# iscc/iscc-search

Measured on AMD Instinct MI355X. Metric: queries/sec (+ roofline of the dominant kernel), 64-bit Hamming k=10 over 100M codes, exact top-k, higher is better.
Workload: dtype fp4 (e2m1 0/1 x +-1 products, f32 accumulation: exact integers)

## Files before the change

### iscc_search_amd/csrc/batch.hip.h

```cpp

void launch_scan(int W, bool mask, int tq, int mode, dim3 grid, hipStream_t st, const isk::ScanParams& p) {
    auto with_tq = [&](auto&& f) { if (tq == 8) f(isk::int_c<8>{}); else f(isk::int_c<16>{}); };
    if (W == 1 && !mask) {
        isk::with_mode(mode, [&](auto m) { with_tq([&](auto t) {
            if constexpr (decltype(m)::value != isk::MODE_SELF) hipLaunchKernelGGL((isk::scan_adapt_kernel<decltype(t)::value, decltype(m)::value>), grid, dim3(isk::BLOCK), 0, st, p);
        }); });
        return;
    }
    isk::with_words(W, [&](auto w) {
        auto masked = [&](auto mk) { with_tq([&](auto t) { isk::with_mode(mode, [&](auto m) {
            constexpr int WORDS = decltype(w)::value, MODE = decltype(m)::value;
            constexpr bool MASK = decltype(mk)::value;
            if constexpr (MODE != isk::MODE_SELF && (WORDS > 1 || MASK)) hipLaunchKernelGGL((isk::scan_kernel<WORDS, MASK, decltype(t)::value, MODE>), grid, dim3(isk::BLOCK), 0, st, p);
        }); }); };
        if (mask) masked(std::true_type{}); else masked(std::false_type{});
    });
}
int tile_rows_for(int W) { return W == 1 ? isk::tile_rows<1>() : W == 2 ? isk::tile_rows<2>() : W == 3 ? isk::tile_rows<3>() : isk::tile_rows<4>(); }

constexpr uint64_t CACHE_RESIDENT_BYTES = 128ull << 20;
uint32_t scan_grid_x(H* h, int W, uint64_t rows, uint32_t groups = 1, bool sample = false) {
    const uint64_t tiles = rows / (uint64_t)tile_rows_for(W);
    uint64_t maxb = (uint64_t)h->cus * BLOCKS_PER_CU;
    if (sample || rows * 8 * (uint64_t)W <= CACHE_RESIDENT_BYTES)
// ... 138 lines not shown
    bool single_pass(const Job& j) const { return allow_self && h->opt.self_tighten && use_mfma(j, j.seg->n); }
    enum class Path { tiny, radius, single, levels };
    Path path(const Job& j) const {
        if (tiny(j)) return Path::tiny;
        if (job_radius(j) >= 0) return Path::radius;
        return single_pass(j) ? Path::single : Path::levels;
    }
    bool pack3(const Job& j) const { return j.pack && h->opt.mfma_pack3 && isk::mfma_pack3_fits(isk::mfma_groups_per_chunk((int)j.W, nq_pad, j.pack)); }
    bool pack3_pass(const Job& j) const { return use_mfma(j, j.seg->n) && pack3(j); }
    int scan(const Job& j, const isk::ScanParams& sp, int mode, bool sample) {
        const uint64_t rows = sp.n_rows - sp.row_begin;
        if (use_mfma(j, rows) || mode == isk::MODE_SELF) {
            const uint32_t g = isk::mfma_groups_per_chunk((int)j.W, nq_pad, j.pack);
            const uint32_t chunks = (nq_pad + g * 32 - 1) / (g * 32);
            const bool pack3 = this->pack3(j);
            const uint64_t rps = isk::mfma_rows_per_wave_step((int)j.W, j.pack, pack3);
            const uint64_t steps = (rows + rps - 1) / rps;
            const uint64_t wpb = isk::mfma_waves_per_block();
            const uint64_t bx = std::max<uint64_t>(1, std::min<uint64_t>((steps + wpb - 1) / wpb, std::max<uint32_t>(1, (uint32_t)h->cus * isk::mfma_blocks_per_cu((int)j.W, g, j.pack) / chunks)));
            const int e = isk::launch_mfma_scan((int)j.W, mode, j.pack, (uint32_t)bx, g, h->stream, sp, pack3);
            if (e) return fail(-EIO, "mfma scan: chunk of %u query groups does not fit the LDS budget (%s)", g, hipGetErrorString((hipError_t)e));
            h->stats.mfma_launches += 1;
            if (j.pack) h->stats.mfma_pack_launches += 1;
            h->stats.mfma_pair_words += rows * (uint64_t)nq * j.W;
            return 0;
        }
        if (mode != isk::MODE_COLLECT && mode != isk::MODE_STRETCH && mode != isk::MODE_BOTH) return fail(-EINVAL, "scan mode %d has no XOR + popcount kernel", mode);
        if (sp.n_rows / (uint64_t)tile_rows_for((int)j.W) >= (1ull << 31)) return fail(-E2BIG, "segment of %llu rows exceeds the scan kernel's 2^31 tiles", (unsigned long long)sp.n_rows);
        launch_scan((int)j.W, j.mask, tq, mode, dim3(scan_grid_x(h, j.W, rows, groups, sample), groups), h->stream, sp);
        return 0;
    }

    void plan(const uint64_t* hq) {
        jobs.clear();
        tq = (int)h->opt.queries_per_pass;
        if (tq == 8 && nq > 8 && nq <= 16) tq = 16;
        nq_pad = (nq + tq - 1) / tq * tq;
        groups = nq_pad / tq;
        for (uint32_t b = 1; b <= ISCCSEARCH_MAX_BYTES; ++b) {
            Segment& s = t.seg[b];
            if (!s.n) continue;
            Job j;
            j.seg = &s;
            j.pbytes = t.metric == ISCCSEARCH_METRIC_NPHD ? std::min(b, qbytes) : b;
            j.W = (j.pbytes + 7) / 8;
            j.mask = (j.pbytes & 7) != 0;
            j.mask_last = mask_for(j.pbytes);
            j.pack = h->opt.mfma_pack && j.W == 1;
            if (j.pack && j.pbytes == 8)
                for (uint32_t q = 0; q < nq && j.pack; ++q) j.pack = hq[(size_t)q * t.max_words] != 0;
            jobs.push_back(j);
        }
    }
    int reserve() {
        cap = std::max<uint32_t>((uint32_t)h->opt.candidate_cap, 16 * k);
        if (h->opt.self_tighten && h->opt.mfma && radius < 0 && radius_ratio < 0) cap = std::max<uint32_t>(cap, 64 * k);
        multi = jobs.size() > 1;
        P = next_pow2(std::max<uint32_t>(std::max<uint32_t>(k, 1024), std::min<uint32_t>(4 * k, 4096)));
        sel_lds = (((size_t)P * 4 + 15) & ~(size_t)15) + (size_t)P * 8 * t.key_words + (d_out_rows ? (size_t)P * 4 : 0);
        int rc;
        if ((rc = h->d_queries.ensure((size_t)nq_pad * 4))) return rc;
        if ((rc = h->d_bias.ensure(nq_pad))) return rc;
        if ((rc = h->d_thr.ensure(nq_pad))) return rc;
        if ((rc = h->d_cnt.ensure((size_t)nq_pad * isk::CNT_STRIDE))) return rc;
        if ((rc = h->d_ghist.ensure((size_t)nq_pad * isk::HB))) return rc;
        if (!d_flags) {
            if ((rc = h->d_overflow.ensure(flag_words()))) return rc;
            d_flags = h->d_overflow.p;
        }
        if ((rc = h->d_cand.ensure((size_t)nq_pad * cap))) return rc;
        if (multi) {
            if ((rc = h->d_lists.ensure(jobs.size() * (size_t)nq * k))) return rc;
            if ((rc = h->d_listcnt.ensure(jobs.size() * (size_t)nq))) return rc;
        }
        return 0;
    }
    const uint64_t* staged() const { return h->p_queries.p + pq_off; }
    bool all_tiny() const {
        for (const Job& j : jobs) if (!tiny(j)) return false;
        return true;
    }
    bool inline_queries() const { return !all_tiny() && radius >= 0 && nq_pad <= isk::INLINE_QUERIES && jobs.size() == 1; }
    bool tiny_inline() const { return all_tiny() && nq_pad <= isk::INLINE_QUERIES; }
    int stage(const uint64_t* hq) {
        int rc;
        if ((rc = wait_staged(h))) return rc;
        if ((rc = h->p_queries.ensure(pq_off + (size_t)nq_pad * 4))) return rc;
        uint64_t* const pq = h->p_queries.p + pq_off;
        memset(pq, 0, (size_t)nq_pad * 4 * 8);
        for (uint32_t q = 0; q < nq; ++q)
            for (int w = 0; w < t.max_words; ++w) pq[(size_t)q * 4 + w] = hq[(size_t)q * t.max_words + w];
        if (!inline_queries() && !tiny_inline()) HIPOK(hipMemcpyAsync(h->d_queries.p, pq, (size_t)nq_pad * 4 * 8, hipMemcpyHostToDevice, h->stream));
        if (mark_overflow) { HIPOK(hipEventRecord(h->ev_staged, h->stream)); h->ev_staged_pending = true; }
        return 0;
    }
    int begin(const uint64_t* hq) {
        plan(hq);
        used_self = false;
        if (jobs.empty()) {
            HIPOK(hipMemsetAsync(d_out_cnt, 0, nq * sizeof(uint32_t), h->stream));
            return 0;
        }
        int rc;
        if ((rc = reserve())) return rc;
        if ((rc = stage(hq))) return rc;
        for (size_t ji = 0; ji < jobs.size(); ++ji) {
            Run run{jobs[ji], make_ctx(ji), job_radius(jobs[ji])};
            switch (path(run.j)) {
                case Path::tiny: rc = run_tiny(run); break;
                case Path::radius: rc = run_radius(run); break;
                case Path::single: used_self = true; rc = run_single(run); break;
                case Path::levels: rc = run_levels(run); break;
            }
            if (rc) return rc;
        }
        return 0;
    }

    void count_scan(const Job& j, uint64_t rows, uint32_t passes) {
        h->stats.scan_launches += 1;
        h->stats.scan_passes += passes;
        h->stats.scan_bytes += rows * 8 * j.W * passes;
        h->stats.scan_pair_words += rows * (uint64_t)nq * j.W;
    }
    int run_tiny(Run& run) {
        const Job& j = run.j;
        const Segment& s = *j.seg;
        isk::TinyParams tp{};
        set_cols(tp.col, s, j.W);
        tp.queries = h->d_queries.p; tp.cand = h->d_cand.p; tp.mask_last = j.mask_last; tp.n_rows = (uint32_t)s.n; tp.W = j.W;
        tp.radius = run.radius; tp.use_inline = tiny_inline() ? 1u : 0u;
        isk::InlineQueries iq;
        if (tp.use_inline) memcpy(iq.w, staged(), (size_t)nq_pad * 4 * 8);
        else memset(iq.w, 0, sizeof iq.w);
        hipEvent_t e1 = nullptr;
        int rc;
        if ((rc = profile_begin(h, e1))) return rc;
        const bool wide = (s.n > 2048 && nq <= (uint32_t)h->cus / 2) || run.c.sl.P >= 2 * (uint64_t)h->opt.select_wide_from || (run.c.sl.P >= (uint64_t)h->opt.select_wide_from && nq <= (uint32_t)h->cus / 2);
        if (wide) launch_tiny_nt<1024>(tp, run.c.sl, iq);
        else launch_tiny_nt<isk::BLOCK>(tp, run.c.sl, iq);
        HIPOK(hipGetLastError());
        if ((rc = profile_end(h, e1))) return rc;
        count_scan(j, s.n, nq);
        return 0;
    }

    int collect(Run& run, uint64_t from, bool self = false) {
        const Job& j = run.j;
        const Segment& s = *j.seg;
        isk::ScanParams& sp = run.c.sp;
        const uint64_t tile_rows = (uint64_t)tile_rows_for((int)j.W);
        uint64_t stretch = s.n;
        const bool shared = use_mfma(j, s.n - from) ? nq_pad > isk::mfma_groups_per_chunk((int)j.W, nq_pad, j.pack) * 32 : groups > 1;
        const uint64_t stretch_bytes = ((uint64_t)h->opt.stretch_mb << 20) * (use_mfma(j, s.n - from) ? (uint64_t)h->opt.mfma_stretch_factor : 1);
        if (shared && stretch_bytes) stretch = std::max<uint64_t>(tile_rows, stretch_bytes / (8 * j.W) / tile_rows * tile_rows);
        for (uint64_t a = from; a < s.n;) {
            const uint64_t b = s.n - a <= stretch + stretch / 4 ? s.n : a + stretch;
            sp.row_begin = a;
            sp.n_rows = b;
            const uint64_t rows = b - a;
            hipEvent_t e1 = nullptr;
            int rcl = 0;
            if ((rcl = profile_begin(h, e1))) return rcl;
            const bool hist_too = run.radius < 0;
            const bool repick = hist_too && b < s.n && !self;
            if (self) {
                if ((rcl = scan(j, sp, isk::MODE_SELF, false))) return rcl;
            } else if (hist_too) {
                if (!run.hist_live) { HIPOK(hipMemsetAsync(h->d_ghist.p, 0, (size_t)nq_pad * isk::HB * sizeof(uint32_t), h->stream)); run.hist_live = true; }
                if ((rcl = scan(j, sp, isk::MODE_STRETCH, false))) return rcl;
            } else {
                if ((rcl = scan(j, sp, isk::MODE_COLLECT, false))) return rcl;
            }
            if ((rcl = profile_end(h, e1))) return rcl;
            if (repick) {
                isk::PickParams pp{h->d_ghist.p, h->d_bias.p, nq, (uint32_t)std::min<uint64_t>(k, b), h->d_cnt.p, h->d_cand.p, cap};
                hipLaunchKernelGGL(isk::pick_kernel, dim3(nq), dim3(isk::BLOCK), 0, h->stream, pp);
            }
            count_scan(j, rows, groups);
            if (use_mfma(j, rows) || self) h->stats.scan_mfma_launches += 1;
            a = b;
        }
        return 0;
    }

    int run_radius(Run& run) {
        if (inline_queries()) {
            isk::InlineQueries iq;
            memcpy(iq.w, staged(), (size_t)nq_pad * 4 * 8);
            hipLaunchKernelGGL(isk::radius_init_inline_kernel, dim3(1), dim3(isk::BLOCK), 0, h->stream,
                               h->d_bias.p, h->d_cnt.p, nq, nq_pad, 0x7FFFFFFFu - (uint32_t)run.radius, h->d_queries.p, iq);
        } else
        hipLaunchKernelGGL(isk::radius_init_kernel, dim3((nq_pad + isk::BLOCK - 1) / isk::BLOCK), dim3(isk::BLOCK), 0, h->stream,
                           h->d_bias.p, h->d_cnt.p, nq, nq_pad, 0x7FFFFFFFu - (uint32_t)run.radius);
        int rc;
        if ((rc = collect(run, 0))) return rc;
        launch_select(run.c.sl, nq);
        HIPOK(hipGetLastError());
        return 0;
    }

    uint64_t sample_rows(const Job& j, bool self) const {
        const uint64_t n = j.seg->n;
        return std::min<uint64_t>(n, self ? std::max<uint64_t>(std::max<uint64_t>((uint64_t)h->opt.self_boot_rows, k), std::min<uint64_t>((uint64_t)h->opt.self_boot_per_k * k, n / 8))
                                          : std::max<uint64_t>(BOOT_ROWS, std::min<uint64_t>(65536, 64ull * k)));
    }
    void boot(Run& run, bool self) {
        const Job& j = run.j;
        isk::BootParams bp{};
        set_cols(bp.col, *j.seg, j.W);
        bp.queries = h->d_queries.p; bp.bias = h->d_bias.p; bp.cnt = h->d_cnt.p; bp.s0 = sample_rows(j, self); bp.nq = nq; bp.k = k; bp.W = j.W; bp.mask_last = j.mask_last;
        bp.thr = self ? h->d_thr.p : nullptr;
        bp.thr_packed = j.pack ? 1u : 0u;
        bp.counts = h->d_ghist.p;
        bp.hint = isk::BOOT_NO_HINT;
        run.hist_live = true;
        const int job_hint = self_hint >= 0 ? self_hint : (radius_ratio >= 0 && ratio_starts_self ? ratio_bits(j) : -1);
        if (self && job_hint >= 0) {
            bp.hint = (uint32_t)job_hint;
            used_hint = true;
            hipLaunchKernelGGL(isk::boot_kernel, dim3(nq_pad), dim3(64), 0, h->stream, bp);
        } else if (nq_pad > 64) {
            isk::with_words((int)j.W, [&](auto w) { hipLaunchKernelGGL(isk::boot_multi_kernel<decltype(w)::value>, dim3(nq_pad / isk::BOOT_QB), dim3(1024), 0, h->stream, bp); });
        } else {
            hipLaunchKernelGGL(isk::boot_kernel, dim3(nq_pad), dim3(1024), 0, h->stream, bp);
        }
    }

    int run_single(Run& run) {
        boot(run, true);
        int rc;
        if ((rc = collect(run, 0, true))) return rc;
        launch_select(run.c.sl, nq);
        HIPOK(hipGetLastError());
        return 0;
    }

    uint64_t level_growth(const Job& j) const {
        uint64_t growth = (groups <= 2 && k <= 64) ? 64 : LEVEL_GROWTH;
        if (use_mfma(j, j.seg->n) && k <= 64) growth = MFMA_LEVEL_GROWTH;
        if (k >= 256) growth = std::min<uint64_t>(growth, 2);
        while (growth > 2 && (uint64_t)k * growth * 5 / 2 > (uint64_t)cap * 9 / 10) growth /= 2;
        return growth;
    }
    int run_levels(Run& run) {
        const Job& j = run.j;
        const Segment& s = *j.seg;
        isk::ScanParams& sp = run.c.sp;
        const uint64_t tile_rows = (uint64_t)tile_rows_for((int)j.W);
        int rc;
        boot(run, false);
        const uint64_t growth = level_growth(j);
        uint64_t done = 0;
        uint64_t reach = sample_rows(j, false);
        for (;;) {
            uint64_t end = reach >= s.n / growth ? s.n : reach * growth;
            if (end < s.n) end = end / tile_rows * tile_rows;
            if (end <= done || end + tile_rows > s.n) end = s.n;
            const bool last = end == s.n;
            if (last) break;
            if (!run.hist_live) {
                HIPOK(hipMemsetAsync(h->d_ghist.p, 0, (size_t)nq_pad * isk::HB * sizeof(uint32_t), h->stream));
                run.hist_live = true;
            }
            sp.row_begin = done;
            sp.n_rows = end;
            {
                hipEvent_t e1 = nullptr;
                if ((rc = profile_begin(h, e1, true))) return rc;
                if ((rc = scan(j, sp, isk::MODE_BOTH, true))) return rc;
                if ((rc = profile_end(h, e1))) return rc;
                h->stats.level_launches += 1;
                h->stats.level_pair_words += (end - done) * (uint64_t)nq * j.W;
                if (use_mfma(j, end - done)) h->stats.level_mfma_launches += 1;
            }
            isk::PickParams pp{h->d_ghist.p, h->d_bias.p, nq, (uint32_t)std::min<uint64_t>(k, end), h->d_cnt.p, h->d_cand.p, cap};
            hipLaunchKernelGGL(isk::pick_kernel, dim3(nq), dim3(isk::BLOCK), 0, h->stream, pp);
            h->stats.sample_bytes += (end - done) * 8 * j.W * groups;
// ... 157 lines not shown
```

### iscc_search_amd/csrc/isccsearch.hip

```cpp
#include <hip/hip_runtime.h>

#include <algorithm>
#include <cerrno>
#include <cstdarg>
#include <cstdio>
#include <cmath>
#include <condition_variable>
#include <cstring>
#include <memory>
#include <mutex>
#include <string>
#include <unordered_map>
#include <thread>
#include <atomic>
#include <functional>
#include <vector>

#include "../../include/isccsearch.h"
#include "kernels.hip.h"
#include "join.hip.h"
#include "mfma_scan.h"
#include "docfreq.h"
#include "simprint_score.h"
#include "asset_score.h"
#include "overlap.h"
#include "segments.h"
#include "keymap.h"

namespace {

thread_local std::string g_last_error;

int fail(int code, const char* fmt, ...) {
    char buf[512];
    va_list ap;
    va_start(ap, fmt);
    vsnprintf(buf, sizeof buf, fmt, ap);
    va_end(ap);
    g_last_error = buf;
    return code;
}

#define HIPOK(expr)                                                                              \
    do {                                                                                         \
        hipError_t e_ = (expr);                                                                  \
        if (e_ != hipSuccess) {                                                                  \
            (void)hipGetLastError();                                                             \
            return fail(e_ == hipErrorOutOfMemory ? -ENOMEM : -EIO, "%s failed: %s (%s:%d)", #expr, \
                        hipGetErrorString(e_), __FILE__, __LINE__);                              \
        }                                                                                        \
    } while (0)

using iskhost::Key;
using iskhost::KeyHash;
using iskhost::KeyMap;
using iskhost::Loc;

struct HintBackoff {
    uint32_t k = 0, skip = 0, penalty = 0;
    bool ready(uint32_t want_k) {
        if (k != want_k) return false;
        if (skip) { skip -= 1; return false; }
        return true;
    }
    void miss() { penalty = std::min<uint32_t>(2 * penalty + 1, 15); skip = penalty - 1; }
};

struct Segment {
    uint32_t nbytes = 0, W = 0;
    uint64_t n = 0, cap = 0;
    uint64_t* col[4] = {nullptr, nullptr, nullptr, nullptr};
    uint64_t* keys = nullptr;
    std::vector<uint64_t> hkeys;
    uint32_t* freq = nullptr;
    uint64_t freq_rows = 0;
    uint32_t freq_dup = 0;
    void touch() { freq_rows = 0; }
    struct SpecHint : HintBackoff {
        uint32_t tau = 0;
        static uint32_t margin(uint32_t want_k) { return want_k >= 64 ? 1u : 2u; }
        void hit(uint32_t worst) { penalty = 0; tau = std::min<uint32_t>(std::max<uint32_t>(worst + margin(k), tau ? tau - 1 : 0), 8 * ISCCSEARCH_MAX_BYTES); }
        void seed(uint32_t new_k, uint32_t worst) { k = new_k; tau = std::min<uint32_t>(worst + margin(new_k), 8 * ISCCSEARCH_MAX_BYTES); }
    } spec[12][5];
    SpecHint& hint(uint32_t nq, uint32_t len) { return spec[nq ? 32 - __builtin_clz(nq) : 0][len % 8 == 0 && len >= 8 && len <= 32 ? len / 8 : 0]; }
};

struct Table {
    bool open = false;
    int metric = 0, key_words = 1, max_bytes = 0, max_words = 0;
    Segment seg[ISCCSEARCH_MAX_BYTES + 1];
    struct RatioHint : HintBackoff {
        double ratio = 0.0;
        void hit(double worst) { penalty = 0; ratio = std::max(worst, ratio - 1.0 / 256.0); }
        void seed(uint32_t new_k, double worst) { k = new_k; ratio = worst; }
    } mspec[12][5];
    RatioHint& mhint(uint32_t nq, uint32_t len) { return mspec[nq ? 32 - __builtin_clz(nq) : 0][len % 8 == 0 && len >= 8 && len <= 32 ? len / 8 : 0]; }
    bool indexed = false;
    KeyMap index;
    uint64_t total = 0;
    uint32_t segments() const {
        uint32_t n = 0;
        for (uint32_t b = 1; b <= ISCCSEARCH_MAX_BYTES; ++b) n += seg[b].n ? 1 : 0;
        return n;
    }
    Segment* sole_segment() {
        Segment* one = nullptr;
        for (uint32_t b = 1; b <= ISCCSEARCH_MAX_BYTES; ++b)
            if (seg[b].n) { if (one) return nullptr; one = &seg[b]; }
        return one;
    }
};

constexpr uint32_t QB_MAX = 1024;
constexpr size_t flag_slots_for(size_t m) { return m + 16; }
constexpr size_t staged_words_for(size_t m) { return (m + 16) * 4; }
struct ResultBlock {
    size_t m, k;
    bool with_records = true, with_extra = false, with_info = false, with_flags = true;
    static constexpr ResultBlock merged(size_t m, size_t k) { return ResultBlock{m, k, true, false, false, false}; }
    constexpr size_t records_bytes() const { return with_records ? m * k * sizeof(isk::Record) : 0; }
    constexpr size_t counts_off() const { return records_bytes(); }
    constexpr size_t flags_off() const { return counts_off() + m * sizeof(uint32_t); }
    constexpr size_t extra_off() const { return flags_off() + (with_flags ? flag_slots_for(m) : 0) * sizeof(uint32_t); }
    constexpr size_t info_off() const { return extra_off() + (with_extra ? m : 0) * sizeof(uint32_t); }
    constexpr size_t bytes() const { return info_off() + (with_info ? isksp::INFO_WORDS : 0) * sizeof(uint32_t); }
    constexpr size_t slice_bytes() const { return (bytes() + 15) & ~(size_t)15; }
    constexpr size_t bytes_with(size_t flag_words) const { return flags_off() + flag_words * sizeof(uint32_t); }
    static uint32_t* words(unsigned char* base, size_t off) { return reinterpret_cast<uint32_t*>(base + off); }
    isk::Record* records(unsigned char* base) const { return reinterpret_cast<isk::Record*>(base); }
    uint32_t* counts(unsigned char* base) const { return words(base, counts_off()); }
    uint32_t* flags(unsigned char* base) const { return words(base, flags_off()); }
    uint32_t* extra(unsigned char* base) const { return words(base, extra_off()); }
    uint32_t* info(unsigned char* base) const { return words(base, info_off()); }
};
constexpr size_t RB_REC = sizeof(isk::Record), RB_W = sizeof(uint32_t);
static_assert(ResultBlock{1, 1}.counts_off() == 1 * 1 * RB_REC && ResultBlock{1, 1}.flags_off() == 1 * 1 * RB_REC + 1 * RB_W &&
              ResultBlock{1, 1}.bytes() == 1 * 1 * RB_REC + (1 + (1 + 16)) * RB_W, "one query, one record");
constexpr ResultBlock RB_SINK{5, 3, false, true, true};
static_assert(RB_SINK.counts_off() == 0 && RB_SINK.flags_off() == 5 * RB_W && RB_SINK.extra_off() == (5 + (5 + 16)) * RB_W &&
              RB_SINK.info_off() == (5 + (5 + 16) + 5) * RB_W && RB_SINK.bytes() == (5 + (5 + 16) + 5 + isksp::INFO_WORDS) * RB_W, "a sink's block");
static_assert(ResultBlock{1024, 10}.counts_off() == 1024 * 10 * RB_REC && ResultBlock{1024, 10}.bytes() == 1024 * 10 * RB_REC + (1024 + (1024 + 16)) * RB_W &&
              ResultBlock{1024, 10}.bytes_with(1024) == 1024 * 10 * RB_REC + (1024 + 1024) * RB_W, "a full batch of lists");
static_assert(ResultBlock{1, 2}.bytes() == 120 && ResultBlock{1, 2}.slice_bytes() == ((1 * 2 * RB_REC + (1 + (1 + 16)) * RB_W + 15) & ~(size_t)15) &&
              ResultBlock::merged(3, 1).slice_bytes() == ((3 * 1 * RB_REC + 3 * RB_W + 15) & ~(size_t)15) && ResultBlock::merged(3, 1).slice_bytes() == 96, "slices of 16 bytes");
constexpr uint64_t CACHE_STRETCH_BYTES = 128ull << 20;
constexpr uint64_t ROW_ALIGN = 2048;

template <typename T, bool PINNED>
struct ScratchBuf {
    T* p = nullptr;
    size_t n = 0;
    ScratchBuf() = default;
    ScratchBuf(const ScratchBuf&) = delete;
    ScratchBuf& operator=(const ScratchBuf&) = delete;
    ~ScratchBuf() { release(); }
    int ensure(size_t need) {
        if (need <= n) return 0;
        release();
        const size_t want = need + need / 4 + (PINNED ? 16 : 0);
        const hipError_t e = PINNED ? hipHostMalloc((void**)&p, want * sizeof(T), hipHostMallocDefault) : hipMalloc((void**)&p, want * sizeof(T));
        if (e != hipSuccess) { p = nullptr; (void)hipGetLastError(); return fail(-ENOMEM, "%s(%zu bytes) failed: %s", PINNED ? "hipHostMalloc" : "hipMalloc", want * sizeof(T), hipGetErrorString(e)); }
        n = want;
        return 0;
    }
    void release() { if (p) (void)(PINNED ? hipHostFree(p) : hipFree(p)); p = nullptr; n = 0; }
};
template <typename T> using DevBuf = ScratchBuf<T, false>;
template <typename T> using PinBuf = ScratchBuf<T, true>;

constexpr size_t DIRECT_RESULT_BYTES = 1 << 20;

uint64_t mask_for(uint32_t pbytes) {
    const uint32_t rem = pbytes & 7;
    return rem ? ~0ULL << (8 * (8 - rem)) : ~0ULL;
}
uint32_t next_pow2(uint32_t v) { uint32_t p = 2; while (p < v) p <<= 1; return p; }
template <typename T>
void set_cols(T (&dst)[4], const Segment& s, uint32_t W) { for (uint32_t w = 0; w < W; ++w) dst[w] = s.col[w]; }
void seg_free(Segment& s) {
    for (auto& c : s.col) { if (c) (void)hipFree(c); c = nullptr; }
    if (s.keys) (void)hipFree(s.keys);
    s.keys = nullptr;
    if (s.freq) (void)hipFree(s.freq);
    s.freq = nullptr;
    s.freq_rows = 0;
    s.n = s.cap = 0;
    s.hkeys.clear();
    s.hkeys.shrink_to_fit();
}

constexpr uint32_t BLOCKS_PER_CU = 8;
constexpr uint64_t BOOT_ROWS = 65536;
constexpr uint64_t LEVEL_GROWTH = 8;
constexpr uint64_t MFMA_LEVEL_GROWTH = 4;
constexpr uint32_t FOLD_TAU = 11;
constexpr uint32_t MFMA_PACK_MIN_QUERIES = 9;
constexpr uint64_t MFMA_FEW_ROWS = 12ull << 20;
constexpr uint32_t SELF_REFRESH_STEPS = 1;
constexpr int RADIUS_BATCH_SLACK = 0;
constexpr uint32_t RADIUS_BATCH_MAX_REPAIRS = 32;

struct Options {
    int64_t queries_per_pass = 8;
    int64_t profile = 0;
    int64_t count_candidates = 0;
    int64_t tiny_rows = 16384;
    int64_t select_wide_from = 2048;
    int64_t stretch_mb = CACHE_STRETCH_BYTES >> 20;
    int64_t mfma_stretch_factor = 3;
    int64_t mfma = 1;
    int64_t mfma_min_queries = 17;
    int64_t mfma_min_rows = 65536;
    int64_t mfma_pack = 1;
    int64_t mfma_pack3 = 1;
    int64_t join_mfma = 1;
    int64_t join_mfma_min_rows = 65536;
    int64_t self_tighten = 1;
    int64_t self_boot_rows = 65536;
    int64_t self_boot_per_k = 1024;
    int64_t self_hint = 1;
    int64_t radius_batches = 1;
    int64_t speculate = 1;
    int64_t spec_max_queries = 128;
    int64_t device_search_hint = -1;
    int64_t candidate_cap = 16384;
};

struct OptionDesc { const char* name; int64_t Options::* field; int64_t min, max; };
constexpr int64_t NO_MAX = INT64_MAX;
const OptionDesc OPTIONS[] = {
    {"queries_per_pass", &Options::queries_per_pass, 8, 16},
    {"profile", &Options::profile, 0, 1},
    {"count_candidates", &Options::count_candidates, 0, 1},
    {"tiny_rows", &Options::tiny_rows, 0, 1 << 20},
    {"select_wide_from", &Options::select_wide_from, 0, 0xFFFFFFFFll},
    {"stretch_mb", &Options::stretch_mb, 0, 65536},
    {"mfma_stretch_factor", &Options::mfma_stretch_factor, 1, 64},
    {"mfma", &Options::mfma, 0, 1},
    {"mfma_min_queries", &Options::mfma_min_queries, 1, 1024},
    {"mfma_min_rows", &Options::mfma_min_rows, 1, NO_MAX},
    {"join_mfma", &Options::join_mfma, 0, 1},
    {"join_mfma_min_rows", &Options::join_mfma_min_rows, 0, NO_MAX},
    {"mfma_pack", &Options::mfma_pack, 0, 1},
    {"mfma_pack3", &Options::mfma_pack3, 0, 1},
    {"self_tighten", &Options::self_tighten, 0, 1},
    {"self_boot_rows", &Options::self_boot_rows, 256, 1 << 20},
    {"self_boot_per_k", &Options::self_boot_per_k, 0, 1 << 20},
    {"self_hint", &Options::self_hint, 0, 1},
    {"radius_batches", &Options::radius_batches, 0, 1},
    {"speculate", &Options::speculate, 0, 1},
    {"spec_max_queries", &Options::spec_max_queries, 0, 1024},
    {"device_search_hint", &Options::device_search_hint, -1, 8 * ISCCSEARCH_MAX_BYTES},
    {"candidate_cap", &Options::candidate_cap, 64, 1 << 22},
};
const OptionDesc* find_option(const char* name) {
    for (const OptionDesc& d : OPTIONS)
        if (!strcmp(d.name, name)) return &d;
    return nullptr;
}

#include "simprint_scratch.hip.h"

}

struct PendingSearch;
struct isccsearch_handle {
    std::mutex mu;
    std::mutex qmu;
    std::condition_variable qcv;
    std::vector<PendingSearch*> pending;
    bool leader_active = false;
    int device = 0;
    int cus = 256;
    hipStream_t stream = nullptr;
    std::vector<std::unique_ptr<Table>> tables;
    Options opt;
    uint16_t* d_rank = nullptr;
    DevBuf<uint64_t> d_queries;
    DevBuf<uint32_t> d_bias, d_cnt, d_ghist, d_overflow, d_listcnt, d_outcnt, d_freq;
    DevBuf<float> d_thr;
    DevBuf<uint64_t> d_cand;
    DevBuf<isk::Record> d_lists, d_final;
    PinBuf<uint64_t> p_queries;
    PinBuf<uint32_t> p_flags;
    DevBuf<unsigned char> d_block;
    PinBuf<unsigned char> p_block;
    DevBuf<uint64_t> d_misc;
    DevBuf<uint64_t> d_misc2;
    SimprintScratch sp;
    DevBuf<isk::Record> d_am_rec, d_am_rec2;
    DevBuf<uint32_t> d_am_cnt, d_am_cnt2, d_am_off;
    DevBuf<iskas::Slot> d_am_slots;
    DevBuf<uint64_t> d_am_ex;
    DevBuf<uint8_t> d_am_hasex;
    DevBuf<double> d_am_tab;
    std::vector<double> am_tab;
    DevBuf<iskas::Item> d_am_scratch;
    PinBuf<unsigned char> p_am_out;
    DevBuf<uint64_t> d_join_keys, d_join_total;
    DevBuf<uint32_t> d_join_ham;
    DevBuf<uint16_t> d_join_pb;
    DevBuf<isk::JoinEmit> d_join_emit;
    DevBuf<uint64_t> d_join_live_keys;
    DevBuf<uint32_t> d_join_live_labels, d_join_row_labels, d_join_parent;
    DevBuf<iskov::Hit> d_ov_hits;
    DevBuf<isccsearch_overlap> d_ov_marks, d_ov_records;
    DevBuf<unsigned char> d_ov_temp;
    DevBuf<uint32_t> d_ov_chunks;
    DevBuf<isksg::RowKey> d_sg_keys;
    DevBuf<uint32_t> d_sg_rows;
    DevBuf<isksg::PairKey> d_sg_pairs;
    DevBuf<isksg::Run> d_sg_runs;
    size_t am_lds_allowed = 0;
    hipEvent_t ev_done = nullptr, ev_staged = nullptr, ev_producer = nullptr;
    bool ev_staged_pending = false;
    std::vector<std::pair<hipEvent_t, hipEvent_t>> ev_pool;
    std::vector<char> ev_level;
    size_t ev_used = 0;
    isccsearch_stats stats{};
    void teardown() {
        (void)hipSetDevice(device);
        if (stream) (void)hipStreamSynchronize(stream);
        for (auto& t : tables)
            if (t) for (auto& s : t->seg) seg_free(s);
        tables.clear();
        if (d_rank) { (void)hipFree(d_rank); d_rank = nullptr; }
        for (auto& ev : ev_pool) { (void)hipEventDestroy(ev.first); (void)hipEventDestroy(ev.second); }
        ev_pool.clear();
        for (hipEvent_t* e : {&ev_done, &ev_staged, &ev_producer}) { if (*e) (void)hipEventDestroy(*e); *e = nullptr; }
        if (stream) { (void)hipStreamDestroy(stream); stream = nullptr; }
    }
    ~isccsearch_handle() { teardown(); }
// ... 159 lines not shown
```

### iscc_search_amd/csrc/search_api.hip.h

```cpp
extern "C" {
static_assert(isksp::MAX_QUERY_SIMPRINTS == ISCCSEARCH_MAX_SCORED_SIMPRINTS, "header and kernels disagree");
struct ScoreSink {
    SimprintScratch& sp;
    int h_max = -1;
    uint32_t dup_limit = 0;
    uint32_t entries = 0;
    uint32_t max_count = 0;
    bool unknown_any = false;
    bool exact = false;
    uint32_t nd = 0, ng = 0;
    bool prepared = false;
    uint32_t* q_count = nullptr;

    bool holds_every_lookup(uint32_t pos, uint32_t m) const { return exact && pos == 0 && m == nd; }
    isk::Record* records(uint32_t pos, uint32_t k) const { return sp.rec.p + (size_t)pos * k; }
    uint32_t* rows(uint32_t pos, uint32_t k) const { return exact ? nullptr : sp.rows.p + (size_t)pos * k; }
    hipError_t queue_behind_select(uint32_t pos, uint32_t m, uint32_t k, const uint32_t* d_cnt, uint32_t* d_info, hipStream_t stream) const;
    void take(uint32_t pos, uint32_t m, uint32_t k, const uint32_t* p_cnt, const uint32_t* p_info);
};

struct SearchOut {
    uint64_t* keys = nullptr; uint32_t* hamming = nullptr; uint16_t* prefix_bits = nullptr; uint32_t* count = nullptr;
    uint32_t* freq = nullptr; uint32_t* collisions = nullptr;
    ScoreSink* sink = nullptr;
    static SearchOut lists(uint64_t* k, uint32_t* h, uint16_t* p, uint32_t* c) { SearchOut o; o.keys = k; o.hamming = h; o.prefix_bits = p; o.count = c; return o; }
    static SearchOut doc_freq(uint32_t* freq, uint32_t* collisions = nullptr) { SearchOut o; o.freq = freq; o.collisions = collisions; return o; }
    static SearchOut to_sink(ScoreSink* sink) { SearchOut o; o.sink = sink; return o; }
};
static bool hints_serve(const isccsearch_handle* h, const Segment* seg, uint32_t k, int radius, bool skip_one_launch) {
    if (!seg || radius >= 0 || k > seg->n) return false;
    const bool one_launch = seg->n <= (uint64_t)h->opt.tiny_rows && seg->n < (uint64_t)h->opt.mfma_min_rows && seg->n <= (uint64_t)h->opt.candidate_cap;
    return !(skip_one_launch && one_launch);
}
static int ready_hint(const isccsearch_handle* h, Segment* seg, uint32_t m, uint32_t len, uint32_t k, bool allowed) {
    return allowed && h->opt.speculate && seg->hint(m, len).ready(k) ? (int)seg->hint(m, len).tau : -1;
}
static bool count_verdict(isccsearch_handle* h, HintBackoff& hint, bool ok) {
    if (ok) h->stats.spec_hits += 1;
    else { h->stats.spec_misses += 1; hint.miss(); }
    return ok;
}
static int appended(isccsearch_handle* h, const Batch& b, uint64_t& sum) {
    std::vector<uint32_t> hc((size_t)b.nq_pad * isk::CNT_STRIDE);
    HIPOK(hipMemcpyAsync(hc.data(), h->d_cnt.p, hc.size() * sizeof(uint32_t), hipMemcpyDeviceToHost, h->stream));
    HIPOK(hipStreamSynchronize(h->stream));
    for (uint32_t i = 0; i < b.nq; ++i) sum += hc[(size_t)i * isk::CNT_STRIDE];
    return 0;
}

enum class Spec { none, radius, self_hint, tight, ratio };
struct LockedCall {
    isccsearch_handle* h; Table& t; uint32_t k; int radius; const SearchOut& out;
    bool may_speculate;
    const std::vector<uint32_t>& order;
    const std::vector<uint64_t>& hq;
};
struct LockedBatch : LockedCall {
    const uint32_t pos, m, len;
    const ResultBlock blk;
    ScoreSink* const sink;
    const uint32_t segments;
    const bool one_copy;
    const bool direct;
    unsigned char* const d_base;
    const isk::Record* const p_rec; const uint32_t* const p_cnt;
    Batch batch;
    Segment* const seg;
    bool hintable = false, mhintable = false;
    Spec spec = Spec::none;
    int tau = -1;
    bool spec_ok = false;
    bool handed_out = false;

    LockedBatch(const LockedCall& c, uint32_t pos_, uint32_t m_, uint32_t len_, const ResultBlock& b)
        : LockedCall(c), pos(pos_), m(m_), len(len_), blk(b), sink(c.out.sink), segments(c.t.segments()), one_copy(segments == 1 && !c.out.freq),
          direct(one_copy && b.bytes() <= DIRECT_RESULT_BYTES && !sink), d_base(direct ? c.h->p_block.p : c.h->d_block.p),
          p_rec(b.records(c.h->p_block.p)), p_cnt(b.counts(c.h->p_block.p)),
          batch(c.h, c.t, m_, len_, c.k, sink ? sink->records(pos_, c.k) : b.records(d_base), b.counts(d_base)), seg(c.t.sole_segment()) {
        batch.radius = radius;
        if (sink) { batch.d_out_rows = sink->rows(pos, k); batch.d_out_kth = blk.extra(d_base); }
        if (one_copy) { batch.d_flags = blk.flags(d_base); batch.h_flags = blk.flags(h->p_block.p); }
    }

    bool runs_pack3() { batch.plan(hq.data()); return batch.jobs.size() == 1 && batch.path(batch.jobs[0]) == Batch::Path::single && batch.pack3_pass(batch.jobs[0]); }
    void choose() {
        hintable = hints_serve(h, seg, k, radius, true) && !out.freq && one_copy;
        const bool small_batch = hintable && m <= (uint32_t)h->opt.spec_max_queries;
        tau = ready_hint(h, seg, m, len, k, hintable && may_speculate && (small_batch || h->opt.self_hint));
        if (tau >= 0) {
            if (small_batch) { spec = Spec::radius; batch.radius = tau; }
            else if (h->opt.radius_batches && !sink && runs_pack3()) {
                spec = Spec::tight;
                batch.radius = std::max(0, tau - (int)Segment::SpecHint::margin(k) + RADIUS_BATCH_SLACK);
            } else { spec = Spec::self_hint; batch.self_hint = tau; }
        }
        mhintable = segments > 1 && radius < 0 && !out.freq && (m <= (uint32_t)h->opt.spec_max_queries || h->opt.self_hint) && k <= t.total;
        if (mhintable && h->opt.speculate && may_speculate && t.mhint(m, len).ready(k)) {
            spec = Spec::ratio;
            batch.radius_ratio = t.mhint(m, len).ratio + 1.0 / 32.0;
            batch.ratio_starts_self = m > (uint32_t)h->opt.spec_max_queries;
        }
    }
    int queue_results() {
        if (out.freq) {
            int rf;
            if ((rf = h->d_freq.ensure(m))) return rf;
            isk::DistinctParams dp{batch.d_out, batch.d_out_cnt, h->d_freq.p, k, (uint32_t)t.key_words};
            hipLaunchKernelGGL(isk::distinct_kernel, dim3(m), dim3(isk::BLOCK), 0, h->stream, dp);
            HIPOK(hipGetLastError());
            if (out.collisions) HIPOK(hipMemcpyAsync(blk.extra(h->p_block.p), batch.d_out_cnt, m * sizeof(uint32_t), hipMemcpyDeviceToHost, h->stream));
            HIPOK(hipMemcpyAsync(blk.counts(h->p_block.p), h->d_freq.p, m * sizeof(uint32_t), hipMemcpyDeviceToHost, h->stream));
            return 0;
        }
        if (direct) return 0;
        if (sink) {
            HIPOK(sink->queue_behind_select(pos, m, k, batch.d_out_cnt, blk.info(d_base), h->stream));
            HIPOK(hipMemcpyAsync(h->p_block.p, h->d_block.p, blk.bytes(), hipMemcpyDeviceToHost, h->stream));
            return 0;
        }
        HIPOK(hipMemcpyAsync(h->p_block.p, h->d_block.p, blk.bytes_with(one_copy ? batch.flag_words() : 0), hipMemcpyDeviceToHost, h->stream));
        return 0;
    }
    int settle() {
        int rs;
        if ((rs = batch.merge())) return rs;
        if ((rs = batch.copy_flags())) return rs;
        if ((rs = queue_results())) return rs;
        HIPOK(hipStreamSynchronize(h->stream));
        return 0;
    }
    double worst_ratio() const {
        double worst = 0.0;
        for (uint32_t i = 0; i < m; ++i) {
            if (p_cnt[i] < k) return -1.0;
            const isk::Record& r = p_rec[(size_t)i * k + k - 1];
            worst = std::max(worst, r.prefix_bits ? (double)r.hamming / (double)r.prefix_bits : 0.0);
        }
        return worst;
    }
    int repair(const std::vector<uint32_t>& short_q) {
        int rr;
        unpack_records(p_rec, p_cnt, m, k, t.key_words, &order[pos], out.keys, out.hamming, out.prefix_bits, out.count);
        uint64_t cand = 0;
        if (h->opt.count_candidates && (rr = appended(h, batch, cand))) return rr;
        const uint32_t ns = (uint32_t)short_q.size();
        std::vector<uint64_t> rq((size_t)ns * t.max_words);
        std::vector<uint32_t> dest(ns);
        for (uint32_t j = 0; j < ns; ++j) {
            memcpy(&rq[(size_t)j * t.max_words], &hq[(size_t)short_q[j] * t.max_words], (size_t)t.max_words * 8);
            dest[j] = order[pos + short_q[j]];
        }
        const ResultBlock rblk{ns, k};
        const bool r_direct = rblk.bytes() <= DIRECT_RESULT_BYTES;
        unsigned char* const r_base = r_direct ? h->p_block.p : h->d_block.p;
        const uint32_t* const rp_cnt = rblk.counts(h->p_block.p);
        Batch rb(h, t, ns, len, k, rblk.records(r_base), rblk.counts(r_base));
        rb.radius = tau;
        rb.on_matrix_cores = true;
        rb.d_flags = rblk.flags(r_base);
        rb.h_flags = rblk.flags(h->p_block.p);
        if ((rr = rb.begin(rq.data()))) return rr;
        if (!r_direct) HIPOK(hipMemcpyAsync(h->p_block.p, h->d_block.p, rblk.bytes_with(rb.flag_words()), hipMemcpyDeviceToHost, h->stream));
        HIPOK(hipStreamSynchronize(h->stream));
        if (h->opt.count_candidates && (rr = appended(h, rb, cand))) return rr;
        spec_ok = rb.complete(rp_cnt, seg->n);
        if (!spec_ok) return 0;
        unpack_records(p_rec, rp_cnt, ns, k, t.key_words, dest.data(), out.keys, out.hamming, out.prefix_bits, out.count);
        handed_out = true;
        h->stats.candidates += cand;
        h->stats.spec_repairs += ns;
        return 0;
    }
    int verify() {
        int rc;
        if (spec == Spec::ratio) spec_ok = batch.complete(p_cnt, k) && worst_ratio() <= batch.radius_ratio;
        else if (spec != Spec::tight) spec_ok = batch.complete(p_cnt, seg->n);
        else {
            std::vector<uint32_t> short_q;
            for (uint32_t i = 0; i < m; ++i) if (p_cnt[i] < k) short_q.push_back(i);
            if (batch.any_flag()) spec_ok = false;
            else if (short_q.empty()) spec_ok = true;
            else if (short_q.size() <= RADIUS_BATCH_MAX_REPAIRS) { if ((rc = repair(short_q))) return rc; }
            else {
                batch.radius = radius; batch.self_hint = tau;
                if ((rc = batch.begin(hq.data()))) return rc;
                if ((rc = settle())) return rc;
                spec_ok = batch.used_hint && batch.complete(p_cnt, seg->n);
            }
        }
        return 0;
    }
    int record() {
        int rc;
        if (h->opt.count_candidates && batch.jobs.size() == 1) {
            if (!handed_out && (rc = appended(h, batch, h->stats.candidates))) return rc;
            h->stats.candidate_batches += 1;
        }
        if (handed_out) {
            uint32_t worst = 0;
            for (uint32_t i = 0; i < m; ++i) {
                const size_t dq = order[pos + i];
                if (out.count[dq]) worst = std::max(worst, out.hamming[dq * k + out.count[dq] - 1]);
            }
            record_hint(seg->hint(m, len), spec_ok, k, worst);
        } else if (hintable && !batch.jobs.empty()) record_hint(seg->hint(m, len), spec_ok, m, k, p_cnt, p_rec, sink ? blk.extra(h->p_block.p) : nullptr);
        if (mhintable) {
            const double worst = worst_ratio();
            if (spec_ok) t.mhint(m, len).hit(worst);
            else if (worst >= 0.0) t.mhint(m, len).seed(k, worst);
        }
        return 0;
    }
    void hand_out() {
        const bool none = batch.jobs.empty();
        if (sink) {
            if (!none) sink->take(pos, m, k, p_cnt, blk.info(h->p_block.p));
        } else if (out.freq) {
            for (uint32_t i = 0; i < m; ++i) out.freq[order[pos + i]] = none ? 0 : p_cnt[i];
            if (out.collisions) for (uint32_t i = 0; i < m; ++i) out.collisions[order[pos + i]] = none ? 0 : blk.extra(h->p_block.p)[i];
        } else if (!handed_out) {
            unpack_records(p_rec, p_cnt, m, k, t.key_words, &order[pos], out.keys, out.hamming, out.prefix_bits, out.count);
        }
    }
    int run() {
        int rc;
        choose();
        if ((rc = batch.begin(hq.data()))) return rc;
        if (spec == Spec::ratio && !batch.multi) {
            spec = Spec::none;
            batch.radius_ratio = -1.0;
            if ((rc = batch.begin(hq.data()))) return rc;
        }
        if (spec == Spec::self_hint && !batch.used_hint) spec = Spec::none;
        if (spec != Spec::none) {
            if ((rc = settle()) || (rc = verify())) return rc;
            HintBackoff& hint = spec == Spec::ratio ? static_cast<HintBackoff&>(t.mhint(m, len)) : seg->hint(m, len);
            if (!count_verdict(h, hint, spec_ok)) {
                batch.radius = radius; batch.self_hint = -1; batch.used_hint = false; batch.radius_ratio = -1.0;
                if ((rc = batch.begin(hq.data()))) return rc;
            }
        }
        if (!spec_ok && (rc = batch.finish(hq.data(), [this] { return queue_results(); }))) return rc;
        if ((rc = record())) return rc;
        hand_out();
        return 0;
    }
};

static int search_locked(isccsearch_handle* h, uint32_t table, uint32_t nq, const uint64_t* q_words, const uint8_t* q_nbytes, uint32_t k,
                         int radius, const SearchOut& out, bool may_speculate = true) {
    Table* tp;
    int rc = get_table(h, table, tp);
    if (rc) return rc;
    Table& t = *tp;
    if ((rc = check_query_lengths(t, nq, q_nbytes))) return rc;
    HIPOK(hipSetDevice(h->device));
    h->stats.queries += nq;

    std::vector<uint32_t> order(nq);
    for (uint32_t q = 0; q < nq; ++q) order[q] = q;
    auto qlen = [&](uint32_t q) -> uint32_t { return (t.metric == ISCCSEARCH_METRIC_NPHD) ? q_nbytes[q] : (uint32_t)t.max_bytes; };
    if (t.metric == ISCCSEARCH_METRIC_NPHD)
        std::stable_sort(order.begin(), order.end(), [&](uint32_t a, uint32_t b) { return q_nbytes[a] < q_nbytes[b]; });

// ... 268 lines not shown
```

### iscc_search_amd/csrc/threshold_kernels.hip.h

```cpp
#pragma once

#include <hip/hip_runtime.h>
#include <stdint.h>

#include "scan_params.hip.h"

namespace isk {

__device__ __forceinline__ void block_find_cut(const uint32_t* hist, uint32_t nbins, uint32_t need,
                                               uint32_t* res, uint32_t& bin, uint32_t& less) {
    const uint32_t tid = threadIdx.x;
    if (tid < 64) {
        uint32_t c[5], s = 0;
#pragma unroll
        for (int j = 0; j < 5; ++j) {
            const uint32_t b = tid * 5 + j;
            c[j] = b < nbins ? hist[b] : 0u;
            s += c[j];
        }
        uint32_t incl = s;
#pragma unroll
        for (int off = 1; off < 64; off <<= 1) {
            const uint32_t t = __shfl_up(incl, off, 64);
            if (tid >= (uint32_t)off) incl += t;
        }
        const uint32_t excl = incl - s;
        const uint32_t total = __shfl(incl, 63, 64);
        if (tid == 0 && total < need) {
            uint32_t last = 0, run = 0, below = 0;
            for (uint32_t b = 0; b < nbins; ++b) { if (hist[b]) { last = b; below = run; } run += hist[b]; }
            res[0] = last; res[1] = below;
        }
        if (total >= need && excl < need && need <= incl) {
            uint32_t run = excl;
#pragma unroll
            for (int j = 0; j < 5; ++j) {
                if (run + c[j] >= need) { res[0] = tid * 5 + j; res[1] = run; break; }
                run += c[j];
            }
        }
    }
    __syncthreads();
    bin = res[0];
    less = res[1];
    __syncthreads();
}

__global__ __launch_bounds__(BLOCK) void radius_init_kernel(uint32_t* bias, uint32_t* cnt, uint32_t nq, uint32_t nq_pad, uint32_t value) {
    const uint32_t q = blockIdx.x * BLOCK + threadIdx.x;
    if (q >= nq_pad) return;
    bias[q] = q < nq ? value : BIAS_NEVER;
    cnt[(uint64_t)q * CNT_STRIDE] = 0;
}

constexpr uint32_t INLINE_QUERIES = 16;
struct InlineQueries { uint64_t w[INLINE_QUERIES * 4]; };
__global__ __launch_bounds__(BLOCK) void radius_init_inline_kernel(uint32_t* bias, uint32_t* cnt, uint32_t nq, uint32_t nq_pad, uint32_t value,
                                                                   uint64_t* queries, const InlineQueries iq) {
    const uint32_t i = threadIdx.x;
    if (i < nq_pad * 4) queries[i] = iq.w[i];
    if (i < nq_pad) {
        bias[i] = i < nq ? value : BIAS_NEVER;
        cnt[(uint64_t)i * CNT_STRIDE] = 0;
    }
}

struct BootParams {
    const uint64_t* col[4];
    const uint64_t* queries;
    uint32_t* bias;
    uint32_t* cnt;
    uint64_t s0;
    uint32_t nq;
    uint32_t k;
    uint32_t W;
    uint64_t mask_last;
    float* thr;
    uint32_t thr_packed;
    uint32_t* counts;
    uint32_t hint;
};
constexpr uint32_t BOOT_NO_HINT = 0xFFFFFFFFu;
__device__ __forceinline__ void store_boot_threshold(const BootParams& p, uint32_t q, int thr, bool never) {
    if (p.thr_packed) reinterpret_cast<uint32_t*>(p.thr)[q] = never ? 0u : pack_threshold(thr);
    else p.thr[q] = never ? -1.0e9f : (float)thr;
}
constexpr uint64_t BOOT_EXACT_ROWS = 4096;
__device__ __forceinline__ uint64_t boot_exact_rows(const BootParams& p) {
    return (p.s0 <= BOOT_EXACT_ROWS || (uint64_t)p.k * 4 > BOOT_EXACT_ROWS) ? p.s0 : BOOT_EXACT_ROWS;
}

template <int W>
__device__ __forceinline__ void boot_tail(const BootParams& p, const uint64_t (&qw)[4], uint64_t s1, uint32_t cut, uint32_t* hist) {
    const uint32_t tid = threadIdx.x, nthr = blockDim.x;
    for (uint64_t r0 = s1 + tid; r0 < p.s0; r0 += 8 * nthr) {
        uint64_t x[8][W];
#pragma unroll
        for (int u = 0; u < 8; ++u) {
            const uint64_t r = r0 + (uint64_t)u * nthr;
            const uint64_t rr = r < p.s0 ? r : s1;
#pragma unroll
            for (int w = 0; w < W; ++w) x[u][w] = p.col[w][rr];
        }
#pragma unroll
        for (int u = 0; u < 8; ++u) {
            uint32_t h = 0;
#pragma unroll
            for (int w = 0; w < W; ++w) {
                uint64_t y = x[u][w] ^ qw[w];
                if (w == W - 1) y &= p.mask_last;
                h += (uint32_t)__builtin_popcountll(y);
            }
            if (h <= cut && r0 + (uint64_t)u * nthr < p.s0) atomicAdd(&hist[h], 1u);
        }
    }
}

__global__ __launch_bounds__(1024) void boot_kernel(const BootParams p) {
    __shared__ uint32_t hist[320];
    __shared__ uint32_t res[2];
    const uint32_t q = blockIdx.x, tid = threadIdx.x, nthr = blockDim.x;
    if (tid == 0) p.cnt[(uint64_t)q * CNT_STRIDE] = 0;
    if (p.counts)
        for (uint32_t i = tid; i < HB; i += nthr) p.counts[(uint64_t)q * HB + i] = 0;
    if (q >= p.nq) {
        if (tid == 0) {
            p.bias[q] = BIAS_NEVER;
            if (p.thr) store_boot_threshold(p, q, 0, true);
        }
        return;
    }
    uint64_t qw[4];
    for (uint32_t w = 0; w < 4; ++w) qw[w] = w < p.W ? p.queries[(uint64_t)q * 4 + w] : 0;
// ... 208 lines not shown
```

Measured before the change: 523,300.

## Hold tight radius across batches and copy staged queries inside init kernel

Radius batches now take their search radius from a held worst-distance value, which only drops after 16 consecutive lower observations, instead of tau minus a margin. This aims to cut repair and fallback passes when the radius is too tight. Verification treats a batch whose radius already reached tau as failed. Separately, for larger radius batches the query upload is dropped: radius_init_kernel reads the pinned host staging buffer directly and writes it to device memory, saving one memcpy call per batch. The cost is zero-copy host reads from a kernel and a different mix of spec failures.

```diff
diff --git a/iscc_search_amd/csrc/batch.hip.h b/iscc_search_amd/csrc/batch.hip.h
--- a/iscc_search_amd/csrc/batch.hip.h
+++ b/iscc_search_amd/csrc/batch.hip.h
@@ -244,6 +244,7 @@
     }
     bool inline_queries() const { return !all_tiny() && radius >= 0 && nq_pad <= isk::INLINE_QUERIES && jobs.size() == 1; }
     bool tiny_inline() const { return all_tiny() && nq_pad <= isk::INLINE_QUERIES; }
+    bool staged_queries() const { return !all_tiny() && radius >= 0 && nq_pad > isk::INLINE_QUERIES && jobs.size() == 1; }
     int stage(const uint64_t* hq) {
         int rc;
         if ((rc = wait_staged(h))) return rc;
@@ -252,7 +253,11 @@
         memset(pq, 0, (size_t)nq_pad * 4 * 8);
         for (uint32_t q = 0; q < nq; ++q)
             for (int w = 0; w < t.max_words; ++w) pq[(size_t)q * 4 + w] = hq[(size_t)q * t.max_words + w];
+        if (staged_queries()) return 0;
         if (!inline_queries() && !tiny_inline()) HIPOK(hipMemcpyAsync(h->d_queries.p, pq, (size_t)nq_pad * 4 * 8, hipMemcpyHostToDevice, h->stream));
+        return mark_staged();
+    }
+    int mark_staged() {
         if (mark_overflow) { HIPOK(hipEventRecord(h->ev_staged, h->stream)); h->ev_staged_pending = true; }
         return 0;
     }
@@ -354,8 +359,9 @@
                                h->d_bias.p, h->d_cnt.p, nq, nq_pad, 0x7FFFFFFFu - (uint32_t)run.radius, h->d_queries.p, iq);
         } else
         hipLaunchKernelGGL(isk::radius_init_kernel, dim3((nq_pad + isk::BLOCK - 1) / isk::BLOCK), dim3(isk::BLOCK), 0, h->stream,
-                           h->d_bias.p, h->d_cnt.p, nq, nq_pad, 0x7FFFFFFFu - (uint32_t)run.radius);
-        int rc;
+                           h->d_bias.p, h->d_cnt.p, nq, nq_pad, 0x7FFFFFFFu - (uint32_t)run.radius, h->d_queries.p, staged_queries() ? staged() : nullptr);
+        int rc;
+        if (staged_queries() && (rc = mark_staged())) return rc;
         if ((rc = collect(run, 0))) return rc;
         launch_select(run.c.sl, nq);
         HIPOK(hipGetLastError());
diff --git a/iscc_search_amd/csrc/isccsearch.hip b/iscc_search_amd/csrc/isccsearch.hip
--- a/iscc_search_amd/csrc/isccsearch.hip
+++ b/iscc_search_amd/csrc/isccsearch.hip
@@ -79,8 +79,11 @@
     struct SpecHint : HintBackoff {
         uint32_t tau = 0;
         static uint32_t margin(uint32_t want_k) { return want_k >= 64 ? 1u : 2u; }
-        void hit(uint32_t worst) { penalty = 0; tau = std::min<uint32_t>(std::max<uint32_t>(worst + margin(k), tau ? tau - 1 : 0), 8 * ISCCSEARCH_MAX_BYTES); }
-        void seed(uint32_t new_k, uint32_t worst) { k = new_k; tau = std::min<uint32_t>(worst + margin(new_k), 8 * ISCCSEARCH_MAX_BYTES); }
+        uint32_t keep = 0, low_run = 0, low_max = 0;
+        void hit(uint32_t worst) { penalty = 0; tau = std::min<uint32_t>(std::max<uint32_t>(worst + margin(k), tau ? tau - 1 : 0), 8 * ISCCSEARCH_MAX_BYTES); hold(worst); }
+        void seed(uint32_t new_k, uint32_t worst) { k = new_k; tau = std::min<uint32_t>(worst + margin(new_k), 8 * ISCCSEARCH_MAX_BYTES); keep = worst; low_run = 0; }
+        void hold(uint32_t worst);
+        int tight_radius() const;
     } spec[12][5];
     SpecHint& hint(uint32_t nq, uint32_t len) { return spec[nq ? 32 - __builtin_clz(nq) : 0][len % 8 == 0 && len >= 8 && len <= 32 ? len / 8 : 0]; }
 };
@@ -199,6 +202,13 @@
 constexpr uint32_t SELF_REFRESH_STEPS = 1;
 constexpr int RADIUS_BATCH_SLACK = 0;
 constexpr uint32_t RADIUS_BATCH_MAX_REPAIRS = 32;
+constexpr uint32_t RADIUS_BATCH_HOLD = 16;
+inline void Segment::SpecHint::hold(uint32_t worst) {
+    if (worst >= keep) { keep = worst; low_run = 0; return; }
+    low_max = low_run ? std::max(low_max, worst) : worst;
+    if (++low_run >= RADIUS_BATCH_HOLD) { keep = low_max; low_run = 0; }
+}
+inline int Segment::SpecHint::tight_radius() const { return (int)std::min<uint32_t>(keep + RADIUS_BATCH_SLACK, tau); }
 
 struct Options {
     int64_t queries_per_pass = 8;
@@ -220,6 +230,7 @@
     int64_t self_boot_per_k = 1024;
     int64_t self_hint = 1;
     int64_t radius_batches = 1;
+    int64_t radius_batch_hold = RADIUS_BATCH_HOLD;
     int64_t speculate = 1;
     int64_t spec_max_queries = 128;
     int64_t device_search_hint = -1;
@@ -248,6 +259,7 @@
     {"self_boot_per_k", &Options::self_boot_per_k, 0, 1 << 20},
     {"self_hint", &Options::self_hint, 0, 1},
     {"radius_batches", &Options::radius_batches, 0, 1},
+    {"radius_batch_hold", &Options::radius_batch_hold, RADIUS_BATCH_HOLD, RADIUS_BATCH_HOLD},
     {"speculate", &Options::speculate, 0, 1},
     {"spec_max_queries", &Options::spec_max_queries, 0, 1024},
     {"device_search_hint", &Options::device_search_hint, -1, 8 * ISCCSEARCH_MAX_BYTES},
diff --git a/iscc_search_amd/csrc/search_api.hip.h b/iscc_search_amd/csrc/search_api.hip.h
--- a/iscc_search_amd/csrc/search_api.hip.h
+++ b/iscc_search_amd/csrc/search_api.hip.h
@@ -91,7 +91,7 @@
             if (small_batch) { spec = Spec::radius; batch.radius = tau; }
             else if (h->opt.radius_batches && !sink && runs_pack3()) {
                 spec = Spec::tight;
-                batch.radius = std::max(0, tau - (int)Segment::SpecHint::margin(k) + RADIUS_BATCH_SLACK);
+                batch.radius = seg->hint(m, len).tight_radius();
             } else { spec = Spec::self_hint; batch.self_hint = tau; }
         }
         mhintable = segments > 1 && radius < 0 && !out.freq && (m <= (uint32_t)h->opt.spec_max_queries || h->opt.self_hint) && k <= t.total;
@@ -180,6 +180,7 @@
             for (uint32_t i = 0; i < m; ++i) if (p_cnt[i] < k) short_q.push_back(i);
             if (batch.any_flag()) spec_ok = false;
             else if (short_q.empty()) spec_ok = true;
+            else if (batch.radius >= tau) spec_ok = false;
             else if (short_q.size() <= RADIUS_BATCH_MAX_REPAIRS) { if ((rc = repair(short_q))) return rc; }
             else {
                 batch.radius = radius; batch.self_hint = tau;
diff --git a/iscc_search_amd/csrc/threshold_kernels.hip.h b/iscc_search_amd/csrc/threshold_kernels.hip.h
--- a/iscc_search_amd/csrc/threshold_kernels.hip.h
+++ b/iscc_search_amd/csrc/threshold_kernels.hip.h
@@ -46,9 +46,17 @@
     __syncthreads();
 }
 
-__global__ __launch_bounds__(BLOCK) void radius_init_kernel(uint32_t* bias, uint32_t* cnt, uint32_t nq, uint32_t nq_pad, uint32_t value) {
+__global__ __launch_bounds__(BLOCK) void radius_init_kernel(uint32_t* bias, uint32_t* cnt, uint32_t nq, uint32_t nq_pad, uint32_t value,
+                                                            uint64_t* queries, const uint64_t* staged) {
     const uint32_t q = blockIdx.x * BLOCK + threadIdx.x;
     if (q >= nq_pad) return;
+    if (staged) {
+        const ulonglong2* src = reinterpret_cast<const ulonglong2*>(staged) + (uint64_t)q * 2;
+        ulonglong2* dst = reinterpret_cast<ulonglong2*>(queries) + (uint64_t)q * 2;
+        const ulonglong2 lo = src[0], hi = src[1];
+        dst[0] = lo;
+        dst[1] = hi;
+    }
     bias[q] = q < nq ? value : BIAS_NEVER;
     cnt[(uint64_t)q * CNT_STRIDE] = 0;
 }
```

Result: faster. 542,400 (median of 6 runs) (+3.7%).
